# Nyro-Robotics/booster_gym

Hardware: AMD Instinct MI355X
Metric: env-steps/sec (whole node), PPO rollout+update, T1 4096 envs/GPU (higher is better)
Workload: dtype f32

## Files before the change

### booster_gym_amd/csrc/bg_stamps.h

```cpp
#pragma once
#ifdef BG_CHAIN_PROBE_STAMPS
#define BG_STAMP_BUFFER(BUF, READER, RECORDS, SLOTS)    \
    __device__ long long BUF[(RECORDS) * 4 * (SLOTS)]; \
    extern "C" int READER(void* dst, size_t bytes) { return (int)hipMemcpyFromSymbol(dst, HIP_SYMBOL(BUF), bytes); }
#define BG_STAMP_LOCALS(SLOTS) long long stamps[SLOTS] = {}
#define BG_STAMP(K) stamps[K] = clock64()
#define BG_STAMP_WALL(K) stamps[K] = wall_clock64()
#define BG_STAMP_FENCED(K) do { __builtin_amdgcn_sched_barrier(0); stamps[K] = clock64(); __builtin_amdgcn_sched_barrier(0); } while (0)
#define BG_STAMP_FLUSH(BUF, SLOTS, OK, RECORD)                                                                                   \
    do {                                                                                                                         \
        if ((threadIdx.x & 63) == 0 && (OK))                                                                                     \
            for (int k_ = 0; k_ < (SLOTS); k_++) BUF[((size_t)(RECORD) * 4 + (threadIdx.x >> 6)) * (SLOTS) + k_] = stamps[k_];  \
    } while (0)
#else
#define BG_STAMP_BUFFER(BUF, READER, RECORDS, SLOTS)
#define BG_STAMP_LOCALS(SLOTS) do { } while (0)
#define BG_STAMP(K) do { } while (0)
#define BG_STAMP_WALL(K) do { } while (0)
#define BG_STAMP_FENCED(K) do { } while (0)
#define BG_STAMP_FLUSH(BUF, SLOTS, OK, RECORD) do { } while (0)
#endif
```

### booster_gym_amd/csrc/bg_wgrad_split.hip

```cpp
#include <hip/hip_runtime.h>

#include <type_traits>

#include "bg_wgrad.h"

constexpr int WS_BLOCK = 16;
constexpr int WS_LDS_FLOATS = 36864;
__device__ float ws_zero_block[WS_BLOCK * 512];

struct Pair3 { unsigned h, m, l; };
__device__ __forceinline__ Pair3 split_pair3(float x0, float x1) {
    const unsigned u0 = __float_as_uint(x0), u1 = __float_as_uint(x1);
    Pair3 o;
    o.h = __builtin_amdgcn_perm(u1, u0, 0x07060302u);
    const float r0 = x0 - __uint_as_float(u0 & 0xffff0000u), r1 = x1 - __uint_as_float(u1 & 0xffff0000u);
    const unsigned v0 = __float_as_uint(r0), v1 = __float_as_uint(r1);
    o.m = __builtin_amdgcn_perm(v1, v0, 0x07060302u);
    const float s0 = r0 - __uint_as_float(v0 & 0xffff0000u), s1 = r1 - __uint_as_float(v1 & 0xffff0000u);
    o.l = __builtin_amdgcn_perm(__float_as_uint(s1), __float_as_uint(s0), 0x07060302u);
    return o;
}
__device__ __forceinline__ void set_dword(u32x4 (&pl)[3], int p, const Pair3& v) {
    pl[0][p] = v.h; pl[1][p] = v.m; pl[2][p] = v.l;
}

struct SplitUnit { unsigned u0, u1, t0, t1; float r0, r1; };
template <int NU>
__device__ __forceinline__ void split_op(int o, SplitUnit (&s)[4], const float (&x)[4], const float (&y)[4], Pair3 (&out)[4], int NG, unsigned sgn) {
    const int k = o % NU;
    SplitUnit& q = s[k];
    switch (o / NU) {
        case 0: {
            const unsigned f = k < NG ? sgn : 0u;
            q.u0 = __float_as_uint(x[k]) ^ f; q.u1 = __float_as_uint(y[k]) ^ f; out[k].h = __builtin_amdgcn_perm(q.u1, q.u0, 0x07060302u);
        } break;
        case 1: q.t0 = q.u0 & 0xffff0000u; break;
        case 2: q.t1 = q.u1 & 0xffff0000u; break;
        case 3: q.r0 = __uint_as_float(q.u0) - __uint_as_float(q.t0); break;
        case 4: q.r1 = __uint_as_float(q.u1) - __uint_as_float(q.t1); break;
        case 5: out[k].m = __builtin_amdgcn_perm(__float_as_uint(q.r1), __float_as_uint(q.r0), 0x07060302u); break;
        case 6: q.t0 = __float_as_uint(q.r0) & 0xffff0000u; break;
        case 7: q.t1 = __float_as_uint(q.r1) & 0xffff0000u; break;
        case 8: q.r0 = q.r0 - __uint_as_float(q.t0); break;
        case 9: q.r1 = q.r1 - __uint_as_float(q.t1); break;
        default: out[k].l = __builtin_amdgcn_perm(__float_as_uint(q.r1), __float_as_uint(q.r0), 0x07060302u); break;
    }
}
template <int TERMS, int NU>
__device__ __forceinline__ void tile_mfmas(f32x16& acc, const u32x4 (&g)[3], const u32x4 (&a)[3], const float (&x)[4], const float (&y)[4], Pair3 (&o)[4], unsigned sgn) {
    constexpr int GP[9] = {2, 1, 2, 0, 1, 2, 0, 1, 0}, AP[9] = {2, 2, 1, 2, 1, 0, 1, 0, 0};
    constexpr int NOPS = 11 * NU;
    SplitUnit s[4];
#pragma unroll
    for (int m = 0; m < TERMS; m++) {
        const int term = 9 - TERMS + m;
        BG_MFMA(acc, g[GP[term]], a[AP[term]]);
#pragma unroll
        for (int op = (m * NOPS) / TERMS; op < ((m + 1) * NOPS) / TERMS; op++) {
            split_op<NU == 0 ? 1 : NU>(op, s, x, y, o, NU - 1, sgn);
        }
        BG_PIN();
    }
}

template <int Cout, int Cin, int TERMS>
__device__ __forceinline__ void wgrad_split_tile(float* lds, int M, const float* __restrict__ G, const float* __restrict__ A,
                                                 float* __restrict__ P, int ntile_ci, int tile0, int tw, int slice, int slices) {
    constexpr int TCI = Cin == 64 ? 2 : 4;
    constexpr int UPG = 4 / TCI;
    typedef float avec __attribute__((ext_vector_type(TCI)));
    const int wave = __builtin_amdgcn_readfirstlane(threadIdx.x >> 6), lane = threadIdx.x & 63, i = lane & 31, h = lane >> 5;
    const int ks = 4 / tw, tl = wave % tw, ksub = wave / tw, tile = tile0 + tl;
    const int tco = tile / ntile_ci, tci = tile % ntile_ci;
    const long NB2 = M / (2 * WS_BLOCK), W = (long)slices * ks, widx = (long)slice * ks + ksub;
    const int b0 = 2 * (int)(NB2 * widx / W), b1 = 2 * (int)(NB2 * (widx + 1) / W), nb = b1 - b0;
    const unsigned sgn = (widx & 1) ? 0x80000000u : 0u;
    auto sg = [&](float v) { return __uint_as_float(__float_as_uint(v) ^ sgn); };
    constexpr int gfl = WS_BLOCK * Cout, afl = WS_BLOCK * Cin, grp_fl = gfl + afl;
    const int buf_fl = ks * grp_fl;
    float* my0 = lds + ksub * grp_fl;
    constexpr int NT = (Cout / 128) * (Cin >= 128 ? Cin / 128 : 1), KS = 4 / NT, NBUF = 3 * KS * grp_fl <= WS_LDS_FLOATS ? 3 : 2;
    constexpr int n_inst = grp_fl / 256, N_MINE = n_inst / NT;
    static_assert(n_inst % NT == 0, "every wave of a group issues the same number of copies");
    auto stage = [&](int blk) {
        const bool real = blk < nb;
        const float* gsrc = real ? G + (size_t)(b0 + blk) * gfl : ws_zero_block;
        const float* asrc = real ? A + (size_t)(b0 + blk) * afl : ws_zero_block;
        float* dst = my0 + (blk % NBUF) * buf_fl;
#pragma unroll
        for (int j = 0; j < N_MINE; j++) {
            const int f = (tl + j * NT) * 256;
            const float* src = f < gfl ? gsrc + f : asrc + (f - gfl);
            __builtin_amdgcn_global_load_lds((const __attribute__((address_space(1))) void*)(src + lane * 4), (__attribute__((address_space(3))) void*)(dst + f), 16, 0, 0);
        }
    };
    const int gofs = (8 * h) * Cout + tco * 128 + 4 * i, aofs = gfl + (8 * h) * Cin + tci * (32 * TCI) + TCI * i;

    f32x16 acc[4][TCI];
#pragma unroll
    for (int t = 0; t < 4; t++)
#pragma unroll
        for (int u = 0; u < TCI; u++)
#pragma unroll
            for (int r = 0; r < 16; r++) acc[t][u][r] = 0.f;
    u32x4 gp[2][4][3], ap[2][TCI][3];

#pragma unroll
    for (int c = 0; c < NBUF; c++) stage(c);
    __builtin_amdgcn_s_waitcnt(0x0F70 | ((NBUF - 1) * N_MINE & 15) | (((NBUF - 1) * N_MINE >> 4) << 14));
    __builtin_amdgcn_s_barrier();
    {
        const float* src = my0;
#pragma unroll
        for (int p = 0; p < 4; p++) {
#pragma unroll
            for (int t = 0; t < 4; t++) set_dword(gp[0][t], p, split_pair3(sg(src[gofs + (2 * p) * Cout + t]), sg(src[gofs + (2 * p + 1) * Cout + t])));
#pragma unroll
            for (int u = 0; u < TCI; u++) set_dword(ap[0][u], p, split_pair3(src[aofs + (2 * p) * Cin + u], src[aofs + (2 * p + 1) * Cin + u]));
        }
    }
    auto block = [&](auto cur_c, const float* src) {
        constexpr int CUR = decltype(cur_c)::value, NXT = 1 - CUR;
        f32x4 gq[2][2]; avec aq[2][2];
        auto rd = [&](int t, int w) {
            gq[w][0] = *reinterpret_cast<const f32x4*>(src + gofs + (2 * t) * Cout); gq[w][1] = *reinterpret_cast<const f32x4*>(src + gofs + (2 * t + 1) * Cout);
            aq[w][0] = *reinterpret_cast<const avec*>(src + aofs + (2 * t) * Cin); aq[w][1] = *reinterpret_cast<const avec*>(src + aofs + (2 * t + 1) * Cin);
        };
        rd(0, 0);
#pragma unroll
        for (int t = 0; t < 4; t++) {
            if (t < 3) rd(t + 1, (t + 1) & 1);
            BG_PIN();
            const f32x4 g0 = gq[t & 1][0], g1 = gq[t & 1][1];
            const avec a0 = aq[t & 1][0], a1 = aq[t & 1][1];
#pragma unroll
            for (int u = 0; u < TCI; u++) {
                float x[4], y[4];
                Pair3 o[4];
#pragma unroll
                for (int k = 0; k < UPG; k++) { x[k] = g0[u * UPG + k]; y[k] = g1[u * UPG + k]; }
                x[UPG] = a0[u]; y[UPG] = a1[u];
                BG_PIN();
                tile_mfmas<TERMS, UPG + 1>(acc[t][u], gp[CUR][t], ap[CUR][u], x, y, o, sgn);
#pragma unroll
                for (int k = 0; k < UPG; k++) set_dword(gp[NXT][u * UPG + k], t, o[k]);
                set_dword(ap[NXT][u], t, o[UPG]);
            }
        }
    };
    using c0 = std::integral_constant<int, 0>; using c1 = std::integral_constant<int, 1>;
    auto top = [&](int c) {
        __builtin_amdgcn_s_waitcnt(0x0F70 | ((NBUF - 2) * N_MINE & 15) | (((NBUF - 2) * N_MINE >> 4) << 14));
        __builtin_amdgcn_s_barrier();
        stage(c + NBUF);
    };
    int nbmax = 0;
    for (int c = 0; c < ks; c++) {
        const long wc = (long)slice * ks + c;
        const int len = 2 * (int)(NB2 * (wc + 1) / W) - 2 * (int)(NB2 * wc / W);
        nbmax = len > nbmax ? len : nbmax;
    }
    for (int b = 0; b < nbmax; b += 2) {
        top(b);
        block(c0{}, my0 + ((b + 1) % NBUF) * buf_fl);
        top(b + 1);
        block(c1{}, my0 + ((b + 2) % NBUF) * buf_fl);
    }
    __builtin_amdgcn_s_waitcnt(0x0F70);
    __syncthreads();
    float (*red)[64 * 16 * 2 * TCI] = reinterpret_cast<float (*)[64 * 16 * 2 * TCI]>(lds);
    float* pt = P + (size_t)slice * Cout * Cin + (size_t)(tco * 128) * Cin + tci * (32 * TCI) + TCI * i;
    const int ipw = 32 / ks;
#pragma unroll
    for (int half = 0; half < 2; half++) {
        if (half) __syncthreads();
#pragma unroll
        for (int tt = 0; tt < 2; tt++)
#pragma unroll
            for (int r = 0; r < 16; r++) {
                avec v;
#pragma unroll
                for (int u = 0; u < TCI; u++) v[u] = acc[2 * half + tt][u][r];
                *reinterpret_cast<avec*>(&red[wave][((tt * 16 + r) * 64 + lane) * TCI]) = v;
            }
        __syncthreads();
        for (int k = 0; k < ipw; k++) {
            const int it = ksub * ipw + k, tt = it >> 4, r = it & 15, idx = ((tt * 16 + r) * 64 + lane) * TCI;
            avec v = *reinterpret_cast<const avec*>(&red[tl][idx]);
            if (((long)slice * ks) & 1) v = -v;
            for (int c = 1; c < ks; c++) {
                const avec w = *reinterpret_cast<const avec*>(&red[tl + tw * c][idx]);
                if (((long)slice * ks + c) & 1) v -= w; else v += w;
            }
            const int row = (r & 3) + 8 * (r >> 2) + 4 * h, t = 2 * half + tt;
            *reinterpret_cast<avec*>(pt + (size_t)(4 * row + t) * Cin) = v;
        }
    }
}

template <int TERMS>
__global__ __launch_bounds__(256, 1) void mlp_wgrad_group_split_kernel(WgradGroup grp) {
    __shared__ __attribute__((aligned(16))) float lds[WS_LDS_FLOATS];
    const int b = blockIdx.x;
    int k = 0;
#pragma unroll
    for (int j = 1; j < WG_MAX_PROBLEMS; j++)
        if (j < grp.np && b >= grp.p[j].wg_begin) k = j;
    const WgradProblem& pr = grp.p[k];
    const int groups = pr.ntiles / pr.tw, local = b - pr.wg_begin, tile0 = (local % groups) * pr.tw, slice = local / groups;
    if (pr.Cout == 256 && pr.Cin == 256) wgrad_split_tile<256, 256, TERMS>(lds, pr.M, pr.G, pr.A, pr.P, pr.ntile_ci, tile0, pr.tw, slice, pr.slices);
    else if (pr.Cout == 128 && pr.Cin == 256) wgrad_split_tile<128, 256, TERMS>(lds, pr.M, pr.G, pr.A, pr.P, pr.ntile_ci, tile0, pr.tw, slice, pr.slices);
    else if (pr.Cout == 128 && pr.Cin == 128) wgrad_split_tile<128, 128, TERMS>(lds, pr.M, pr.G, pr.A, pr.P, pr.ntile_ci, tile0, pr.tw, slice, pr.slices);
    else wgrad_split_tile<256, 64, TERMS>(lds, pr.M, pr.G, pr.A, pr.P, pr.ntile_ci, tile0, pr.tw, slice, pr.slices);
}

static int split_launch(const bg_wgrad_problem* problems, int32_t count, int32_t terms, void* stream, bool finish) {
    if (terms != 9 && terms != 6) return bg_set_error(-4, "bg_mlp_weight_grad_group_split: terms must be 9 or 6");
    WgradGroup grp;
    int wg = 0, fin = 0;
    const int rc = bg_wgrad_group_fill(problems, count, grp, wg, fin, "bg_mlp_weight_grad_group_split");
    if (rc) return rc;
    for (int k = 0; k < count; k++) {
        const WgradProblem& p = grp.p[k];
        if (p.tw != p.ntiles) return bg_set_error(-4, "bg_mlp_weight_grad_group_split: tiles_per_workgroup must equal the layer's tile count (1, 2 or 4)");
        if (p.M % (2 * WS_BLOCK) != 0) return bg_set_error(-4, "bg_mlp_weight_grad_group_split: M must be a multiple of 32");
        if ((long)p.slices * (4 / p.tw) > p.M / (2 * WS_BLOCK)) return bg_set_error(-4, "bg_mlp_weight_grad_group_split: too many slices for M");
        if ((4 / p.tw) * WS_BLOCK * (p.Cout + p.Cin) * 2 > WS_LDS_FLOATS) return bg_set_error(-4, "bg_mlp_weight_grad_group_split: layer too wide for the LDS staging");
        const bool known = (p.Cout == 256 && (p.Cin == 256 || p.Cin == 64)) || (p.Cout == 128 && (p.Cin == 256 || p.Cin == 128));
        if (!known) return bg_set_error(-4, "bg_mlp_weight_grad_group_split: unsupported shape (256 x 256, 128 x 256, 128 x 128, 256 x 64)");
    }
    hipStream_t st = (hipStream_t)stream;
    if (terms == 9) hipLaunchKernelGGL(mlp_wgrad_group_split_kernel<9>, dim3(wg), dim3(256), 0, st, grp);
    else hipLaunchKernelGGL(mlp_wgrad_group_split_kernel<6>, dim3(wg), dim3(256), 0, st, grp);
    if (finish && bg_wgrad_group_finish_launch(grp, fin, st)) return bg_set_error(-2, "bg_mlp_weight_grad_group_split: launch failed");
    HIP_OK(hipGetLastError());
    return 0;
}

extern "C" int bg_mlp_weight_grad_group_split(const bg_wgrad_problem* problems, int32_t count, int32_t terms, void* stream) {
    return split_launch(problems, count, terms, stream, true);
}
extern "C" int bg_mlp_weight_grad_group_split_partial(const bg_wgrad_problem* problems, int32_t count, int32_t terms, void* stream) {
    return split_launch(problems, count, terms, stream, false);
}
```

Before: 4.615 million.

## Interleave wgrad LDS staging copies into MFMA schedule via buffer loads

```diff
diff --git a/booster_gym_amd/csrc/bg_stamps.h b/booster_gym_amd/csrc/bg_stamps.h
--- a/booster_gym_amd/csrc/bg_stamps.h
+++ b/booster_gym_amd/csrc/bg_stamps.h
@@ -7,9 +7,14 @@
 #define BG_STAMP(K) stamps[K] = clock64()
 #define BG_STAMP_WALL(K) stamps[K] = wall_clock64()
 #define BG_STAMP_FENCED(K) do { __builtin_amdgcn_sched_barrier(0); stamps[K] = clock64(); __builtin_amdgcn_sched_barrier(0); } while (0)
+#define BG_STAMP_OPEN(K) do { __builtin_amdgcn_sched_barrier(0); stamps[K] -= clock64(); __builtin_amdgcn_sched_barrier(0); } while (0)
+#define BG_STAMP_CLOSE(K) do { __builtin_amdgcn_sched_barrier(0); stamps[K] += clock64(); __builtin_amdgcn_sched_barrier(0); } while (0)
+#define BG_STAMP_TURN(K, L) do { __builtin_amdgcn_sched_barrier(0); const long long t_ = clock64(); stamps[K] += t_; stamps[L] -= t_; __builtin_amdgcn_sched_barrier(0); } while (0)
+#define BG_STAMP_WALL_OPEN(K) stamps[K] -= wall_clock64()
+#define BG_STAMP_WALL_CLOSE(K) stamps[K] += wall_clock64()
 #define BG_STAMP_FLUSH(BUF, SLOTS, OK, RECORD)                                                                                   \
     do {                                                                                                                         \
-        if ((threadIdx.x & 63) == 0 && (OK))                                                                                     \
+        if ((threadIdx.x & 63) == 0 && (OK))                                                                                   \
             for (int k_ = 0; k_ < (SLOTS); k_++) BUF[((size_t)(RECORD) * 4 + (threadIdx.x >> 6)) * (SLOTS) + k_] = stamps[k_];  \
     } while (0)
 #else
@@ -18,5 +23,10 @@
 #define BG_STAMP(K) do { } while (0)
 #define BG_STAMP_WALL(K) do { } while (0)
 #define BG_STAMP_FENCED(K) do { } while (0)
+#define BG_STAMP_OPEN(K) do { } while (0)
+#define BG_STAMP_CLOSE(K) do { } while (0)
+#define BG_STAMP_TURN(K, L) do { } while (0)
+#define BG_STAMP_WALL_OPEN(K) do { } while (0)
+#define BG_STAMP_WALL_CLOSE(K) do { } while (0)
 #define BG_STAMP_FLUSH(BUF, SLOTS, OK, RECORD) do { } while (0)
 #endif
diff --git a/booster_gym_amd/csrc/bg_wgrad_split.hip b/booster_gym_amd/csrc/bg_wgrad_split.hip
--- a/booster_gym_amd/csrc/bg_wgrad_split.hip
+++ b/booster_gym_amd/csrc/bg_wgrad_split.hip
@@ -3,10 +3,12 @@
 #include <type_traits>
 
 #include "bg_wgrad.h"
+#include "bg_stamps.h"
 
 constexpr int WS_BLOCK = 16;
 constexpr int WS_LDS_FLOATS = 36864;
 __device__ float ws_zero_block[WS_BLOCK * 512];
+BG_STAMP_BUFFER(bg_wgrad_split_stamp_buf, bg_probe_read_wgrad_split_stamps, 1024, 5)
 
 struct Pair3 { unsigned h, m, l; };
 __device__ __forceinline__ Pair3 split_pair3(float x0, float x1) {
@@ -46,8 +48,9 @@
         default: out[k].l = __builtin_amdgcn_perm(__float_as_uint(q.r1), __float_as_uint(q.r0), 0x07060302u); break;
     }
 }
-template <int TERMS, int NU>
-__device__ __forceinline__ void tile_mfmas(f32x16& acc, const u32x4 (&g)[3], const u32x4 (&a)[3], const float (&x)[4], const float (&y)[4], Pair3 (&o)[4], unsigned sgn) {
+template <int TERMS, int NU, class Copy>
+__device__ __forceinline__ void tile_mfmas(f32x16& acc, const u32x4 (&g)[3], const u32x4 (&a)[3], const float (&x)[4], const float (&y)[4], Pair3 (&o)[4], unsigned sgn,
+                                           int pj, Copy copy) {
     constexpr int GP[9] = {2, 1, 2, 0, 1, 2, 0, 1, 0}, AP[9] = {2, 2, 1, 2, 1, 0, 1, 0, 0};
     constexpr int NOPS = 11 * NU;
     SplitUnit s[4];
@@ -55,6 +58,7 @@
     for (int m = 0; m < TERMS; m++) {
         const int term = 9 - TERMS + m;
         BG_MFMA(acc, g[GP[term]], a[AP[term]]);
+        if (m == 0 && pj >= 0) copy(pj);
 #pragma unroll
         for (int op = (m * NOPS) / TERMS; op < ((m + 1) * NOPS) / TERMS; op++) {
             split_op<NU == 0 ? 1 : NU>(op, s, x, y, o, NU - 1, sgn);
@@ -62,6 +66,24 @@
         BG_PIN();
     }
 }
+
+template <int TCI, int N, int NBUF>
+struct CopySchedule {
+    static constexpr int NG = 4 * TCI, USABLE = NBUF >= 3 ? NG : NG / 2, DEALT = N < USABLE ? N : USABLE, BURST = N - DEALT;
+    static constexpr int cls(int g) { return g % TCI == 0 ? 2 : (g % TCI) & 1 ? 0 : 1; }
+    static constexpr bool dealt(int g) {
+        if (g >= USABLE) return false;
+        int rank = 0;
+        for (int o = 0; o < USABLE; o++) rank += cls(o) < cls(g) || (cls(o) == cls(g) && o < g);
+        return rank < DEALT;
+    }
+    static constexpr int piece(int g) {
+        if (!dealt(g)) return -1;
+        int j = BURST;
+        for (int o = 0; o < g; o++) j += dealt(o);
+        return j;
+    }
+};
 
 template <int Cout, int Cin, int TERMS>
 __device__ __forceinline__ void wgrad_split_tile(float* lds, int M, const float* __restrict__ G, const float* __restrict__ A,
@@ -69,6 +91,7 @@
     constexpr int TCI = Cin == 64 ? 2 : 4;
     constexpr int UPG = 4 / TCI;
     typedef float avec __attribute__((ext_vector_type(TCI)));
+    BG_STAMP_LOCALS(5);
     const int wave = __builtin_amdgcn_readfirstlane(threadIdx.x >> 6), lane = threadIdx.x & 63, i = lane & 31, h = lane >> 5;
     const int ks = 4 / tw, tl = wave % tw, ksub = wave / tw, tile = tile0 + tl;
     const int tco = tile / ntile_ci, tci = tile % ntile_ci;
@@ -82,17 +105,25 @@
     constexpr int NT = (Cout / 128) * (Cin >= 128 ? Cin / 128 : 1), KS = 4 / NT, NBUF = 3 * KS * grp_fl <= WS_LDS_FLOATS ? 3 : 2;
     constexpr int n_inst = grp_fl / 256, N_MINE = n_inst / NT;
     static_assert(n_inst % NT == 0, "every wave of a group issues the same number of copies");
+    constexpr int NG_MINE = gfl / 256 / NT;
+    static_assert((gfl / 256) % NT == 0, "a wave's piece j is G's or A's for every wave of the group");
+    using Sched = CopySchedule<TCI, N_MINE, NBUF>;
+    const int sub_bytes = nb * WS_BLOCK * 4;
+    const __amdgpu_buffer_rsrc_t rs_g = __builtin_amdgcn_make_buffer_rsrc(const_cast<float*>(G + (size_t)b0 * gfl), 0, sub_bytes * Cout, 0x00020000);
+    const __amdgpu_buffer_rsrc_t rs_a = __builtin_amdgcn_make_buffer_rsrc(const_cast<float*>(A + (size_t)b0 * afl), 0, sub_bytes * Cin, 0x00020000);
+    const __amdgpu_buffer_rsrc_t rs_z = __builtin_amdgcn_make_buffer_rsrc(ws_zero_block, 0, (int)sizeof(ws_zero_block), 0x00020000);
+    const int lane16 = lane * 16;
+    auto piece = [&](int blk, int j) {
+        const bool real = blk < nb, is_g = j < NG_MINE;
+        const int q = tl + j * NT;
+        const int in_op = is_g ? q * 1024 : q * 1024 - gfl * 4;
+        const int soff = real ? blk * ((is_g ? gfl : afl) * 4) + in_op : in_op;
+        float* dst = my0 + (blk % NBUF) * buf_fl + q * 256;
+        __builtin_amdgcn_raw_ptr_buffer_load_lds(real ? (is_g ? rs_g : rs_a) : rs_z, (__attribute__((address_space(3))) void*)dst, 16, lane16, soff, 0, 0);
+    };
     auto stage = [&](int blk) {
-        const bool real = blk < nb;
-        const float* gsrc = real ? G + (size_t)(b0 + blk) * gfl : ws_zero_block;
-        const float* asrc = real ? A + (size_t)(b0 + blk) * afl : ws_zero_block;
-        float* dst = my0 + (blk % NBUF) * buf_fl;
-#pragma unroll
-        for (int j = 0; j < N_MINE; j++) {
-            const int f = (tl + j * NT) * 256;
-            const float* src = f < gfl ? gsrc + f : asrc + (f - gfl);
-            __builtin_amdgcn_global_load_lds((const __attribute__((address_space(1))) void*)(src + lane * 4), (__attribute__((address_space(3))) void*)(dst + f), 16, 0, 0);
-        }
+#pragma unroll
+        for (int j = 0; j < N_MINE; j++) piece(blk, j);
     };
     const int gofs = (8 * h) * Cout + tco * 128 + 4 * i, aofs = gfl + (8 * h) * Cin + tci * (32 * TCI) + TCI * i;
 
@@ -119,7 +150,7 @@
             for (int u = 0; u < TCI; u++) set_dword(ap[0][u], p, split_pair3(src[aofs + (2 * p) * Cin + u], src[aofs + (2 * p + 1) * Cin + u]));
         }
     }
-    auto block = [&](auto cur_c, const float* src) {
+    auto block = [&](auto cur_c, const float* src, int cblk) {
         constexpr int CUR = decltype(cur_c)::value, NXT = 1 - CUR;
         f32x4 gq[2][2]; avec aq[2][2];
         auto rd = [&](int t, int w) {
@@ -141,7 +172,7 @@
                 for (int k = 0; k < UPG; k++) { x[k] = g0[u * UPG + k]; y[k] = g1[u * UPG + k]; }
                 x[UPG] = a0[u]; y[UPG] = a1[u];
                 BG_PIN();
-                tile_mfmas<TERMS, UPG + 1>(acc[t][u], gp[CUR][t], ap[CUR][u], x, y, o, sgn);
+                tile_mfmas<TERMS, UPG + 1>(acc[t][u], gp[CUR][t], ap[CUR][u], x, y, o, sgn, Sched::piece(t * TCI + u), [&](int j) { piece(cblk, j); });
 #pragma unroll
                 for (int k = 0; k < UPG; k++) set_dword(gp[NXT][u * UPG + k], t, o[k]);
                 set_dword(ap[NXT][u], t, o[UPG]);
@@ -150,9 +181,15 @@
     };
     using c0 = std::integral_constant<int, 0>; using c1 = std::integral_constant<int, 1>;
     auto top = [&](int c) {
+        BG_PIN();
+        BG_STAMP_OPEN(0);
         __builtin_amdgcn_s_waitcnt(0x0F70 | ((NBUF - 2) * N_MINE & 15) | (((NBUF - 2) * N_MINE >> 4) << 14));
         __builtin_amdgcn_s_barrier();
-        stage(c + NBUF);
+        BG_STAMP_TURN(0, 1);
+#pragma unroll
+        for (int j = 0; j < Sched::BURST; j++) piece(c + NBUF, j);
+        BG_STAMP_CLOSE(1);
+        BG_PIN();
     };
     int nbmax = 0;
     for (int c = 0; c < ks; c++) {
@@ -160,12 +197,16 @@
         const int len = 2 * (int)(NB2 * (wc + 1) / W) - 2 * (int)(NB2 * wc / W);
         nbmax = len > nbmax ? len : nbmax;
     }
+    BG_STAMP_WALL_OPEN(4);
+    BG_STAMP_OPEN(2);
     for (int b = 0; b < nbmax; b += 2) {
         top(b);
-        block(c0{}, my0 + ((b + 1) % NBUF) * buf_fl);
+        block(c0{}, my0 + ((b + 1) % NBUF) * buf_fl, b + NBUF);
         top(b + 1);
-        block(c1{}, my0 + ((b + 2) % NBUF) * buf_fl);
-    }
+        block(c1{}, my0 + ((b + 2) % NBUF) * buf_fl, b + 1 + NBUF);
+    }
+    BG_STAMP_TURN(2, 3);
+    BG_STAMP_WALL_CLOSE(4);
     __builtin_amdgcn_s_waitcnt(0x0F70);
     __syncthreads();
     float (*red)[64 * 16 * 2 * TCI] = reinterpret_cast<float (*)[64 * 16 * 2 * TCI]>(lds);
@@ -196,6 +237,8 @@
             *reinterpret_cast<avec*>(pt + (size_t)(4 * row + t) * Cin) = v;
         }
     }
+    BG_STAMP_CLOSE(3);
+    BG_STAMP_FLUSH(bg_wgrad_split_stamp_buf, 5, blockIdx.x < 1024, blockIdx.x);
 }
 
 template <int TERMS>
```

Result: faster. 4.685 million (median of 6 runs) (+1.5%).
